# pengpeng-yu/FastPCC

Hardware: AMD Instinct MI355X
Metric: encode+decode Mpoints/sec, lossy_coord_v2 baseline_r1 (stream of 16-frame batches, 2 in flight; one frame at a time = value_one_frame) (higher is better)
Workload: dtype f32; 1 GPU; lossy_coord_v2/baseline_r1 inference, 997645-voxel 1024^3 body-surface frames (cfg#2), seeded random-init weights; one step = a batch of 16 such frames per GPU (15966320 voxels) through compress_many + decompress_many = ONE network traversal over the batch, 16 independent streams; 2 batch(es) in flight per GPU; parallelism=single GPU, 2 batches in flight per GPU on one stream (fastpcc_amd/serving.py), batch_clouds=16, frames_in_flight=2, named_stages=False, bytes=143901, coder_handover_retries=0

## Files before the change

fastpcc_amd/csrc/hip/conv.hip:

```cpp
#include "conv_common.h"
#include <atomic>
#include <cstdlib>

namespace fpcc {
namespace {

template <int NBT, int CH, int WM, int WN>
struct MfmaCfg {
    static constexpr int C_OUT = 32 * NBT;
    static constexpr int TM = 32 * WM;
    static constexpr int NBW = NBT / WN;
    static constexpr int THREADS = 64 * WM * WN;
    static constexpr int G8 = CH / 8;
    static constexpr int W_TOTAL = CH * C_OUT / 4;
    static constexpr int W_PIECES = (W_TOTAL + THREADS - 1) / THREADS;
    static_assert(NBT % WN == 0, "column blocks must divide over the waves");
};

template <typename C, int CH>
__device__ __forceinline__ void fetch_a(const ConvArgs &a, const int32_t *nbr_rows, int cc, int li, int lh,
                                        f32x4 (&ra)[C::G8]) {
    const bool in_x1 = cc * CH < a.c1;
    const float *xb = in_x1 ? a.x1 + cc * CH : a.x2 + (cc * CH - a.c1);
    const int64_t ld = in_x1 ? a.ld1 : a.ld2;
// ... 610 lines not shown
            for (int r = 0; r < 16; ++r) acc[rb][nb][r] = 0.0f;

    const int n_stages = __popc(wmask) * n_chunks;
    if (n_stages > 0) {
        const int64_t chunk_floats = (int64_t)G8 * nbt * 256;
        const float *wp_g = wp + (int64_t)g * a.n_off * n_chunks * chunk_floats + ((int64_t)cg * 2) * 256 + lane * 4;
        const float *const zero = (const float *)g_zero_row + 4 * lh;
        const float *const x1b = a.x1 + 4 * lh, *const x2b = a.x2 ? a.x2 + 4 * lh : zero;
        const int64_t ld1 = a.ld1, ld2 = a.ld2;
        const int n1 = a.c1 / CH;
        const float *a1[2], *a2[2], *bpk;
        int step[2];
        auto set_offset = [&](int k) {
#pragma unroll
            for (int rb = 0; rb < 2; ++rb) {
                const int32_t idx = s_nbr[k * 64 + 32 * rb + li];
                const int32_t neg = idx >> 31;
                const uint64_t m = (uint64_t)(int64_t)neg, z = reinterpret_cast<uint64_t>(zero) & m;
                const int64_t row = idx & ~neg;
                a1[rb] = reinterpret_cast<const float *>((reinterpret_cast<uint64_t>(x1b + row * ld1) & ~m) | z);
                a2[rb] = reinterpret_cast<const float *>((reinterpret_cast<uint64_t>(x2b + row * ld2) & ~m) | z);
                step[rb] = CH & ~neg;
            }
            bpk = wp_g + (int64_t)k * n_chunks * chunk_floats;
        };
        unsigned rest = wmask;
        int cc_f = 0;
        set_offset(__ffs(rest) - 1);
        const float *ap[2], *bp;
        auto next_stage = [&]() {
            const bool in1 = cc_f < n1;
            const int c = in1 ? cc_f : cc_f - n1;
            ap[0] = (in1 ? a1[0] : a2[0]) + c * step[0];
            ap[1] = (in1 ? a1[1] : a2[1]) + c * step[1];
            bp = bpk + cc_f * chunk_floats;
            if (cc_f + 1 < n_chunks) {
                ++cc_f;
            } else {
                const unsigned r2 = rest & (rest - 1);
                if (r2) { rest = r2; cc_f = 0; set_offset(__ffs(r2) - 1); }
            }
        };
        f32x4 ra[2][G8], rbv[G8][2];
        next_stage();
#pragma unroll
        for (int g8 = 0; g8 < G8; ++g8) {
            __builtin_amdgcn_sched_barrier(0);
            ra[0][g8] = *reinterpret_cast<const f32x4 *>(ap[0] + 8 * g8);
            __builtin_amdgcn_sched_barrier(0);
            ra[1][g8] = *reinterpret_cast<const f32x4 *>(ap[1] + 8 * g8);
#pragma unroll
            for (int nb = 0; nb < 2; ++nb) {
                __builtin_amdgcn_sched_barrier(0);
                rbv[g8][nb] = *reinterpret_cast<const f32x4 *>(bp + ((int64_t)g8 * nbt + nb) * 256);
            }
        }
        __builtin_amdgcn_sched_barrier(0);
        for (int s = 0; s < n_stages; ++s) {
            next_stage();
            __builtin_amdgcn_sched_barrier(SB);
#pragma unroll
            for (int g8 = 0; g8 < G8; ++g8) {
                const f32x4 av0 = ra[0][g8], av1 = ra[1][g8];
                const f32x4 b0 = rbv[g8][0], b1 = rbv[g8][1];
#define FPCC_STEP(c)                                                                                     \
                acc[0][0] = __builtin_amdgcn_mfma_f32_32x32x2f32(av0.c, b0.c, acc[0][0], 0, 0, 0);       \
                acc[0][1] = __builtin_amdgcn_mfma_f32_32x32x2f32(av0.c, b1.c, acc[0][1], 0, 0, 0);       \
                acc[1][0] = __builtin_amdgcn_mfma_f32_32x32x2f32(av1.c, b0.c, acc[1][0], 0, 0, 0);       \
                acc[1][1] = __builtin_amdgcn_mfma_f32_32x32x2f32(av1.c, b1.c, acc[1][1], 0, 0, 0);
                FPCC_STEP(x) FPCC_STEP(y) FPCC_STEP(z) FPCC_STEP(w)
#undef FPCC_STEP
                __builtin_amdgcn_sched_barrier(SB);
                ra[0][g8] = *reinterpret_cast<const f32x4 *>(ap[0] + 8 * g8);
                __builtin_amdgcn_sched_barrier(SB);
                ra[1][g8] = *reinterpret_cast<const f32x4 *>(ap[1] + 8 * g8);
#pragma unroll
                for (int nb = 0; nb < 2; ++nb) {
                    __builtin_amdgcn_sched_barrier(SB);
                    rbv[g8][nb] = *reinterpret_cast<const f32x4 *>(bp + ((int64_t)g8 * nbt + nb) * 256);
                }
                __builtin_amdgcn_sched_barrier(SB);
            }
        }
    }

    const float slope = (a.act == FPCC_ACT_PRELU && a.slope) ? a.slope[0] : 0.0f;
    float bias2[2];
#pragma unroll
    for (int nb = 0; nb < 2; ++nb) bias2[nb] = a.bias ? a.bias[32 * ((int)cg * 2 + nb) + li] : 0.0f;
#pragma unroll
    for (int rb = 0; rb < 2; ++rb) {
        int64_t dsts[16];
#pragma unroll
        for (int reg = 0; reg < 16; ++reg) {
            const int64_t o = __shfl(my_row, 32 * rb + (reg & 3) + 8 * (reg >> 2) + 4 * lh);
            dsts[reg] = o < 0 ? -1 : a.out_map ? (int64_t)a.out_map[o * a.om_os + g * a.om_gs] : o * a.groups + g;
        }
#pragma unroll
        for (int reg = 0; reg < 16; ++reg) {
            const int64_t dst = dsts[reg];
            if (dst < 0) continue;
#pragma unroll
            for (int nb = 0; nb < 2; ++nb)
                a.out[dst * a.ldo + 32 * ((int)cg * 2 + nb) + li] = finish(acc[rb][nb][reg], bias2[nb], a.act, slope, a.clip);
        }
    }
}

__global__ __launch_bounds__(256) void k_pack_weights(const float *__restrict__ w, int64_t n_mats, int c_in, int c_out,
                                                      float *__restrict__ wp) {
    const int64_t e = (int64_t)blockIdx.x * 256 + threadIdx.x;
    const int64_t per_mat = (int64_t)c_in * c_out;
    if (e >= n_mats * per_mat) return;
    const int nbt = c_out / 32;
    const int64_t m = e / per_mat;
    int64_t r = e - m * per_mat;
    const int j = (int)(r & 3); r >>= 2;
    const int i = (int)(r & 31); r >>= 5;
    const int h = (int)(r & 1); r >>= 1;
    const int nb = (int)(r % nbt); r /= nbt;
    const int g8 = (int)(r & 3); r >>= 2;
    const int cc = (int)r;
    wp[e] = w[m * per_mat + (int64_t)(32 * cc + 8 * g8 + 4 * h + j) * c_out + 32 * nb + i];
}

inline bool aligned16(const void *p) { return (reinterpret_cast<uintptr_t>(p) & 15) == 0; }

int mfma_chunk(int c1, int c2, int c_out) {
    if (c_out != 32 && c_out != 64 && c_out != 128) return 0;
    const int c_in = c1 + c2;
    if (c_in % 32 == 0 && c1 % 32 == 0) return 32;
    if (c_in % 16 == 0 && c1 % 16 == 0) return 16;
    return 0;
}

int knob(int k);

template <int NBT, int CH, int WM, int WN>
int launch_mfma_cfg(ConvArgs a, hipStream_t s) {
    constexpr int TM = 32 * WM;
    const unsigned tiles = (unsigned)((a.n_out + TM - 1) / TM);
    const dim3 grid(tiles, a.groups), block(64 * WM * WN);
    const int dbg = (NBT == 4 && CH == 32) ? knob(3) : 0;
    if (dbg == 1) hipLaunchKernelGGL((k_conv_mfma<NBT, CH, WM, WN, 1>), grid, block, 0, s, a);
    else if (dbg == 2) hipLaunchKernelGGL((k_conv_mfma<NBT, CH, WM, WN, 2>), grid, block, 0, s, a);
    else if (dbg == 3) hipLaunchKernelGGL((k_conv_mfma<NBT, CH, WM, WN, 3>), grid, block, 0, s, a);
    else if (dbg == 4) hipLaunchKernelGGL((k_conv_mfma<NBT, CH, WM, WN, 4>), grid, block, 0, s, a);
    else if (dbg == 7) hipLaunchKernelGGL((k_conv_mfma<NBT, CH, WM, WN, 7>), grid, block, 0, s, a);
    else hipLaunchKernelGGL((k_conv_mfma<NBT, CH, WM, WN>), grid, block, 0, s, a);
    return check_hip(hipGetLastError(), "k_conv_mfma");
}

enum { kKnobWaveOn = 0, kKnobWaveNbw = 1, kKnobWaveSb = 2, kKnobWaveDbg = 3, kKnobGroupedFoldRows = 4, kKnobMfmaCfg = 5, kKnobPointwiseRows = 6,
       kKnobGroupedOff = 7, kKnobGroupedNbw = 8, kKnobWave22Rows = 9, kKnobLdsRows = 10, kKnobLdsRowBlocks = 11, kKnobPersist = 12, kKnobCount = 13 };
int g_knob[kKnobCount] = {-1, -1, -1, -1, -1, -1, -1, -1, -1, -1, -1, -1, -1};
int knob(int k) {
    if (g_knob[k] < 0) {
        static const char *names[kKnobCount] = {"FPCC_CONV_WAVE", "FPCC_WAVE_NBW", "FPCC_WAVE_SB", "FPCC_WAVE_DBG", "FPCC_GROUPED_FOLD_ROWS",
                                                "FPCC_MFMA_TILE", "FPCC_POINTWISE_MIN_ROWS", "", "FPCC_GROUPED_NBW",
                                                "FPCC_WAVE22_MIN_ROWS", "FPCC_LDS_MIN_ROWS", "FPCC_LDS_ROW_BLOCKS",
                                                "FPCC_CONV_PERSIST"};
        static const int defaults[kKnobCount] = {1, 0, 1, 0, 100 * 1024, 0, 32 * 1024, 0, 0, 0, 0, 2, 0};
        const char *e = k == kKnobGroupedOff ? nullptr : getenv(names[k]);
        g_knob[k] = e ? atoi(e) : defaults[k];
    }
    return g_knob[k];
}

template <int NBT, int CH>
int launch_mfma(const ConvArgs &a, hipStream_t s) {
    const int forced = knob(kKnobMfmaCfg) - 1;
    const int64_t work = a.n_out * a.groups;
    constexpr int WNS = NBT >= 2 ? 2 : 1;
    const int cfg = forced >= 0 ? forced : (NBT <= 2 && work >= 128 * 1024) ? 0 : work >= 32 * 1024 ? 1 : 2;
    if (cfg == 0) return launch_mfma_cfg<NBT, CH, 4, 1>(a, s);
    if (cfg == 1) return launch_mfma_cfg<NBT, CH, 2, WNS>(a, s);
    return launch_mfma_cfg<NBT, CH, 1, NBT>(a, s);
}

__global__ __launch_bounds__(256) void k_conv_c1_pointwise(ConvArgs a) {
    const int64_t e = (int64_t)blockIdx.x * 256 + threadIdx.x;
    if (e >= a.n_out * a.c_out) return;
    const int64_t o = e / a.c_out;
    const int j = (int)(e - o * a.c_out);
    const float slope = (a.act == FPCC_ACT_PRELU && a.slope) ? a.slope[0] : 0.0f;
    a.out[o * a.ldo + j] = finish(fmaf(a.x1[o * a.ld1], a.w[j], 0.0f), a.bias ? a.bias[j] : 0.0f, a.act, slope, a.clip);
}

template <int NBW>
int launch_wave_cfg(const ConvArgs &a, const float *wp, int nbt, hipStream_t s) {
    const int64_t row_blocks = (a.n_out + 31) / 32;
    const int64_t units = row_blocks * (nbt / NBW);
    if (units > 0x7fffffffll) return fail_arg("conv_f32: too many work units");
    const dim3 grid((unsigned)((units + 3) / 4), a.groups);
    const int dbg = knob(kKnobWaveDbg);
    if (dbg == 1) hipLaunchKernelGGL((k_conv_wave<NBW, 32, 0x6, 1>), grid, dim3(256), 0, s, a, wp, nbt, (unsigned)units);
    else if (dbg == 2) hipLaunchKernelGGL((k_conv_wave<NBW, 32, 0x6, 2>), grid, dim3(256), 0, s, a, wp, nbt, (unsigned)units);
    else if (dbg == 3) hipLaunchKernelGGL((k_conv_wave<NBW, 32, 0x6, 3>), grid, dim3(256), 0, s, a, wp, nbt, (unsigned)units);
    else if (knob(kKnobWaveSb)) hipLaunchKernelGGL((k_conv_wave<NBW, 32, 0x6>), grid, dim3(256), 0, s, a, wp, nbt, (unsigned)units);
    else hipLaunchKernelGGL((k_conv_wave<NBW, 32, 0>), grid, dim3(256), 0, s, a, wp, nbt, (unsigned)units);
    return check_hip(hipGetLastError(), "k_conv_wave");
}

constexpr int kMaxDevices = 16;
inline int current_device() {
    int dev = 0;
    return (hipGetDevice(&dev) == hipSuccess && dev >= 0 && dev < kMaxDevices) ? dev : -1;
}
int cu_count() {
    static std::atomic<int> cached[kMaxDevices];
    const int dev = current_device();
    if (dev < 0) return 256;
    int n = cached[dev].load(std::memory_order_relaxed);
    if (n == 0) {
        hipDeviceProp_t prop;
        n = (hipGetDeviceProperties(&prop, dev) == hipSuccess && prop.multiProcessorCount > 0) ? prop.multiProcessorCount : 256;
        cached[dev].store(n, std::memory_order_relaxed);
    }
    return n;
}

constexpr int kUnitCounters = 256;
__device__ unsigned g_unit_counters[kUnitCounters];
unsigned *next_unit_counter(unsigned start, hipStream_t s, int *rc) {
    static std::atomic<unsigned> seq{0};
    static std::atomic<unsigned *> bases[kMaxDevices];
    const int dev = current_device();
    if (dev < 0) {
        *rc = fail_arg("unit counters: no current device");
        return nullptr;
    }
    unsigned *base = bases[dev].load(std::memory_order_acquire);
    if (!base) {
        if (hipGetSymbolAddress(reinterpret_cast<void **>(&base), HIP_SYMBOL(g_unit_counters)) != hipSuccess) {
            *rc = check_hip(hipGetLastError(), "unit counters");
            return nullptr;
        }
        bases[dev].store(base, std::memory_order_release);
    }
    unsigned *c = base + (seq++ % kUnitCounters);
    *rc = check_hip(hipMemsetD32Async(reinterpret_cast<hipDeviceptr_t>(c), (int)start, 1, s), "unit counter fill");
    return c;
}

inline int64_t persist_slots() {
    const int v = knob(kKnobPersist);
    return v > 16 ? v : (int64_t)v * cu_count();
}
inline bool persist_ok(const ConvArgs &a) {
    return knob(kKnobPersist) > 0 && a.nbr && a.nbr_ks == 1 && (a.nbr_os & 3) == 0 && a.nbr_os >= ((a.n_off + 3) & ~3) &&
           (reinterpret_cast<uintptr_t>(a.nbr) & 15) == 0 && a.groups == 1;
}

template <int NBW>
int launch_grouped_cfg(const ConvArgs &a, const float *wp, int nbt, hipStream_t s) {
    const int64_t row_blocks = (a.n_out + 31) / 32;
    const int64_t units = row_blocks * (nbt / NBW);
    if (units > 0x7fffffffll) return fail_arg("conv_f32: too many work units");
    const int dbg = knob(kKnobWaveDbg);
    const int64_t slots = persist_slots();
    if (dbg == 0 && persist_ok(a) && units > slots) {
        int rc = FPCC_OK;
        unsigned *counter = next_unit_counter((unsigned)slots, s, &rc);
        if (rc != FPCC_OK) return rc;
        hipLaunchKernelGGL((k_conv_wave<NBW, 32, 0x6, 0, 4, false, false, true>), dim3((unsigned)slots, 1), dim3(256), 0, s, a, wp, nbt, (unsigned)units,
                           counter);
        return check_hip(hipGetLastError(), "k_conv_wave(grouped, persistent)");
    }
    if (dbg == 16)
        hipLaunchKernelGGL((k_conv_wave<NBW, 32, 0x6, 16, 4>), dim3((unsigned)units, a.groups), dim3(256), 0, s, a, wp, nbt, (unsigned)units);
    else if (NBW == 1 && dbg == 17)
        hipLaunchKernelGGL((k_conv_wave<1, 32, 0x6, 17, 4>), dim3((unsigned)units, a.groups), dim3(256), 0, s, a, wp, nbt, (unsigned)units);
    else if (NBW == 1 && dbg == 18)
        hipLaunchKernelGGL((k_conv_wave<1, 32, 0x6, 18, 4>), dim3((unsigned)units, a.groups), dim3(256), 0, s, a, wp, nbt, (unsigned)units);
    else if (NBW == 1 && dbg == 19)
        hipLaunchKernelGGL((k_conv_wave<1, 32, 0x6, 19, 4>), dim3((unsigned)units, a.groups), dim3(256), 0, s, a, wp, nbt, (unsigned)units);
    else
        hipLaunchKernelGGL((k_conv_wave<NBW, 32, 0x6, 0, 4>), dim3((unsigned)units, a.groups), dim3(256), 0, s, a, wp, nbt, (unsigned)units);
    return check_hip(hipGetLastError(), "k_conv_wave(grouped)");
}

template <int NBW>
int launch_folded_cfg(const ConvArgs &a, const float *wp, int nbt, hipStream_t s) {
    const int64_t units = ((a.n_out + 31) / 32) * (nbt / NBW);
    if (units > 0x7fffffffll) return fail_arg("conv_f32: too many work units");
    const int64_t slots = persist_slots();
    if (knob(kKnobWaveDbg) == 0 && persist_ok(a) && (units + 3) / 4 > slots) {
        int rc = FPCC_OK;
        unsigned *counter = next_unit_counter((unsigned)(4 * slots), s, &rc);
        if (rc != FPCC_OK) return rc;
        hipLaunchKernelGGL((k_conv_wave<NBW, 32, 0x6, 0, 1, true, false, true>), dim3((unsigned)slots, 1), dim3(256), 0, s, a, wp, nbt, (unsigned)units,
                           counter);
        return check_hip(hipGetLastError(), "k_conv_wave(folded, persistent)");
    }
    if (knob(kKnobWaveDbg) == 64) {
        hipLaunchKernelGGL((k_conv_wave<NBW, 32, 0x6, 0, 1, true, false, false, 1>), dim3((unsigned)units, a.groups), dim3(64), 0, s, a, wp, nbt,
                           (unsigned)units);
        return check_hip(hipGetLastError(), "k_conv_wave(folded, one wave per workgroup)");
    }
    if (NBW == 2 && knob(kKnobWaveDbg) == 32)
        hipLaunchKernelGGL((k_conv_wave<2, 32, 0x6, 0, 1, true, true>), dim3((unsigned)((units + 3) / 4), a.groups), dim3(256), 0, s, a, wp, nbt,
                           (unsigned)units);
    else
        hipLaunchKernelGGL((k_conv_wave<NBW, 32, 0x6, 0, 1, true>), dim3((unsigned)((units + 3) / 4), a.groups), dim3(256), 0, s, a, wp, nbt,
                           (unsigned)units);
    return check_hip(hipGetLastError(), "k_conv_wave(folded)");
}

int launch_grouped(const ConvArgs &a, const float *wp, hipStream_t s) {
    const int nbt = a.c_out / 32;
    const int64_t lds_rows = knob(kKnobLdsRows);
    if (lds_rows > 0 && a.n_out >= lds_rows) {
        const int rc = launch_conv_lds(a, wp, knob(kKnobLdsRowBlocks), knob(kKnobWaveDbg) & 63, s);
        if (rc != -1) return rc;
    }
    const int64_t fold_rows = knob(kKnobGroupedFoldRows);
    if (fold_rows > 0 && a.n_out >= fold_rows && knob(kKnobGroupedNbw) <= 0)
        return nbt % 2 == 0 ? launch_folded_cfg<2>(a, wp, nbt, s) : launch_folded_cfg<1>(a, wp, nbt, s);
    int nbw = knob(kKnobGroupedNbw);
    if (nbw <= 0) nbw = a.n_out >= 40 * 1024 ? 2 : 1;
    while (nbw > nbt || nbt % nbw) nbw >>= 1;
    return nbw == 2 ? launch_grouped_cfg<2>(a, wp, nbt, s) : launch_grouped_cfg<1>(a, wp, nbt, s);
}

int launch_wave22(const ConvArgs &a, const float *wp, int nbt, hipStream_t s) {
    const int64_t units = ((a.n_out + 63) / 64) * (nbt / 2);
    if (units > 0x7fffffffll) return fail_arg("conv_f32: too many work units");
    const dim3 grid((unsigned)((units + 3) / 4), a.groups);
    if (knob(kKnobWaveSb)) hipLaunchKernelGGL((k_conv_wave22<0x6>), grid, dim3(256), 0, s, a, wp, nbt, (unsigned)units);
    else hipLaunchKernelGGL((k_conv_wave22<0>), grid, dim3(256), 0, s, a, wp, nbt, (unsigned)units);
    return check_hip(hipGetLastError(), "k_conv_wave22");
}

int launch_wave(const ConvArgs &a, const float *wp, hipStream_t s) {
    const int nbt = a.c_out / 32;
    const int64_t work = a.n_out * a.groups;
    const int64_t rows22 = knob(kKnobWave22Rows);
    if (rows22 > 0 && a.n_off > 1 && nbt % 2 == 0 && work >= rows22 && knob(kKnobWaveNbw) <= 0) return launch_wave22(a, wp, nbt, s);
    int nbw = knob(kKnobWaveNbw);
    if (nbw <= 0) nbw = work >= 32 * 1024 ? 2 : 1;
    while (nbw > nbt || nbt % nbw) nbw >>= 1;
    if (nbw >= 4) return launch_wave_cfg<4>(a, wp, nbt, s);
    if (nbw == 2) return launch_wave_cfg<2>(a, wp, nbt, s);
    return launch_wave_cfg<1>(a, wp, nbt, s);
}


template <int NBW, int NCH, int DBG = 0>
__global__ __launch_bounds__(256, 2) void k_pointwise_wave(ConvArgs a, const float *__restrict__ wp, int nbt, unsigned n_row_blocks,
                                                           unsigned waves_per_cg) {
    constexpr int AC = NCH < 4 ? NCH : 4;
    constexpr int TW = 32 * NBW + 4;
    __shared__ float s_tile[4][32 * TW];
    const int lane = threadIdx.x & 63, wv = threadIdx.x >> 6;
    const int li = lane & 31, lh = lane >> 5;
    const unsigned n_cg = (unsigned)(nbt / NBW);
    const unsigned w = blockIdx.x * 4u + (unsigned)wv;
    const unsigned cg = w % n_cg, slot = w / n_cg;
    if (slot >= waves_per_cg) return;

    f32x4 rb[NCH][4][NBW];
    {
        const float *wpl = wp + ((int64_t)cg * NBW) * 256 + lane * 4;
#pragma unroll
        for (int cc = 0; cc < NCH; ++cc)
#pragma unroll
            for (int g8 = 0; g8 < 4; ++g8)
#pragma unroll
                for (int nb = 0; nb < NBW; ++nb)
                    rb[cc][g8][nb] = *reinterpret_cast<const f32x4 *>(wpl + (((int64_t)cc * 4 + g8) * nbt + nb) * 256);
    }
    const int n1 = a.c1 / 32;
    const float slope = (a.act == FPCC_ACT_PRELU && a.slope) ? a.slope[0] : 0.0f;
    float bias[NBW];
#pragma unroll
    for (int nb = 0; nb < NBW; ++nb) bias[nb] = a.bias ? a.bias[32 * ((int)cg * NBW + nb) + li] : 0.0f;

    auto row_ptrs = [&](unsigned rbk, const float *&q1, const float *&q2) {
        int64_t row = (int64_t)rbk * 32 + li;
        if (row >= a.n_out) row = a.n_out - 1;
        if (DBG & 1) row = lane & 1;
        q1 = a.x1 + row * a.ld1 + 4 * lh;
        q2 = a.x2 ? a.x2 + row * a.ld2 + 4 * lh : q1;
    };
    auto fetch = [&](const float *q1, const float *q2, int cc, int g8) -> f32x4 {
        if (DBG & 8) { const float v = (float)(lane + g8 + cc); return f32x4{v, v + 1.0f, v + 2.0f, v + 3.0f}; }
        const float *src = cc < n1 ? q1 + 32 * cc : q2 + 32 * (cc - n1);
        return *reinterpret_cast<const f32x4 *>(src + 8 * g8);
    };
    const float *c1p, *c2p, *n1p, *n2p;
    row_ptrs(slot, c1p, c2p);
    f32x4 ra[AC][4];
#pragma unroll
    for (int c = 0; c < AC; ++c)
#pragma unroll
        for (int g8 = 0; g8 < 4; ++g8) {
            __builtin_amdgcn_sched_barrier(0);
            ra[c][g8] = fetch(c1p, c2p, c, g8);
        }
    __builtin_amdgcn_sched_barrier(0);
    for (unsigned rbk = slot; rbk < n_row_blocks; rbk += waves_per_cg) {
        const int64_t row0 = (int64_t)rbk * 32;
        row_ptrs(rbk + waves_per_cg, n1p, n2p);
        f32x16 acc[NBW];
#pragma unroll
        for (int nb = 0; nb < NBW; ++nb)
#pragma unroll
            for (int r = 0; r < 16; ++r) acc[nb][r] = 0.0f;
#pragma unroll
        for (int cc = 0; cc < NCH; ++cc) {
            constexpr int kNone = 0;
            (void)kNone;
            const int sl = cc % AC;
            const bool wraps = cc + AC >= NCH;
            const int cn = (cc + AC) % NCH;
#pragma unroll
            for (int g8 = 0; g8 < 4; ++g8) {
                const f32x4 av = ra[sl][g8];
#pragma unroll
                for (int nb = 0; nb < NBW; ++nb) acc[nb] = __builtin_amdgcn_mfma_f32_32x32x2f32(av.x, rb[cc][g8][nb].x, acc[nb], 0, 0, 0);
#pragma unroll
                for (int nb = 0; nb < NBW; ++nb) acc[nb] = __builtin_amdgcn_mfma_f32_32x32x2f32(av.y, rb[cc][g8][nb].y, acc[nb], 0, 0, 0);
#pragma unroll
                for (int nb = 0; nb < NBW; ++nb) acc[nb] = __builtin_amdgcn_mfma_f32_32x32x2f32(av.z, rb[cc][g8][nb].z, acc[nb], 0, 0, 0);
#pragma unroll
                for (int nb = 0; nb < NBW; ++nb) acc[nb] = __builtin_amdgcn_mfma_f32_32x32x2f32(av.w, rb[cc][g8][nb].w, acc[nb], 0, 0, 0);
                __builtin_amdgcn_sched_barrier(0x6);
                ra[sl][g8] = wraps ? fetch(n1p, n2p, cn, g8) : fetch(c1p, c2p, cn, g8);
                __builtin_amdgcn_sched_barrier(0x6);
            }
        }
        c1p = n1p;
        c2p = n2p;
        float *tile = s_tile[wv];
#pragma unroll
        for (int reg = 0; reg < 16; ++reg) {
            const int r = (reg & 3) + 8 * (reg >> 2) + 4 * lh;
#pragma unroll
            for (int nb = 0; nb < NBW; ++nb) tile[r * TW + 32 * nb + li] = finish(acc[nb][reg], bias[nb], a.act, slope, a.clip);
        }
        __builtin_amdgcn_wave_barrier();
        constexpr int LPR = 8 * NBW;
        constexpr int RPI = 64 / LPR;
        const int qr = lane / LPR, qc = lane % LPR;
#pragma unroll
        for (int r0 = 0; r0 < 32; r0 += RPI) {
            const int r = r0 + qr;
            const f32x4 v = *reinterpret_cast<const f32x4 *>(tile + r * TW + 4 * qc);
            const int64_t o = row0 + r;
            if (o < a.n_out && !((DBG & 4) && v.x != 12345.678f))
                *reinterpret_cast<f32x4 *>(a.out + o * a.ldo + 32 * (int)cg * NBW + 4 * qc) = v;
        }
        __builtin_amdgcn_wave_barrier();
    }
}


template <int NBW, int NCH>
int launch_pointwise_cfg(const ConvArgs &a, const float *wp, int nbt, hipStream_t s) {
    const unsigned row_blocks = (unsigned)((a.n_out + 31) / 32);
    const unsigned n_cg = (unsigned)(nbt / NBW);
    unsigned waves_per_cg = (256u * 4u * 2u) / n_cg;
    if (waves_per_cg > row_blocks) waves_per_cg = row_blocks;
    const unsigned waves = waves_per_cg * n_cg;
    const int dbg = (NBW == 2 && NCH == 4) ? knob(kKnobWaveDbg) : 0;
    if (dbg == 1) hipLaunchKernelGGL((k_pointwise_wave<NBW, NCH, 1>), dim3((waves + 3) / 4), dim3(256), 0, s, a, wp, nbt, row_blocks, waves_per_cg);
// ... 582 lines not shown
```

fastpcc_amd/csrc/hip/conv_common.h:

```cpp
#pragma once
#include "common.h"

namespace fpcc {

typedef float f32x16 __attribute__((ext_vector_type(16)));
typedef float f32x4 __attribute__((ext_vector_type(4)));

struct ConvArgs {
    const float *x1; int c1; int ld1;
    const float *x2; int c2; int ld2;
    const int32_t *nbr; int n_off; int64_t nbr_ks; int64_t nbr_os;
    const float *w; const float *bias; int c_out; int groups;
    const int32_t *out_map; int64_t om_os; int64_t om_gs; float *out; int ldo; int64_t n_out;
    int act; const float *slope; float clip;
    const int32_t *row_order;
};

static __device__ float g_zero_row[64];

__device__ __forceinline__ float finish(float v, float b, int act, float slope, float clip) {
    v = v + b;
    if (act == FPCC_ACT_PRELU) v = v < 0.0f ? v * slope : v;
    else if (act == FPCC_ACT_RELU) v = v < 0.0f ? 0.0f : v;
    if (clip > 0.0f) v = fminf(fmaxf(v, -clip), clip);
    return v;
}

__device__ __forceinline__ unsigned xcd_remap(unsigned bid, unsigned n) {
    const unsigned q = n / 8, r = n % 8, x = bid % 8;
    return (x < r ? x * (q + 1) : r * (q + 1) + (x - r) * q) + bid / 8;
}

constexpr int kMaxOffsets = 27;

typedef int i32x4 __attribute__((ext_vector_type(4)));

__device__ __forceinline__ bool table_is_row_major(const ConvArgs &a) {
    return a.nbr && a.nbr_ks == 1 && (a.nbr_os & 3) == 0 && a.nbr_os >= ((a.n_off + 3) & ~3) && (reinterpret_cast<uintptr_t>(a.nbr) & 15) == 0;
}

__host__ __device__ __forceinline__ int offset_group_begin(int g, int n_off) { return (g * n_off + 3) / 4; }
__host__ __device__ __forceinline__ int offset_group_of(int k, int n_off) {
    return (k >= offset_group_begin(1, n_off)) + (k >= offset_group_begin(2, n_off)) + (k >= offset_group_begin(3, n_off));
}

constexpr int kStampSlots = 48;
static __device__ unsigned long long *g_stamp_buf = nullptr;
static __device__ long long g_stamp_cap = 0;
__device__ __forceinline__ void stamp_lds(unsigned long long *slot) {
    const unsigned long long t = __builtin_amdgcn_s_memtime();
    const unsigned addr = (unsigned)(uintptr_t)slot;
    asm volatile("s_mov_b64 exec, 1\n\tds_write_b64 %0, %1\n\ts_mov_b64 exec, -1" ::"v"(addr), "v"(t) : "memory");
}
__device__ __forceinline__ void stamp_lds_realtime(unsigned long long *slot) {
    const unsigned long long t = __builtin_amdgcn_s_memrealtime();
    const unsigned addr = (unsigned)(uintptr_t)slot;
    asm volatile("s_mov_b64 exec, 1\n\tds_write_b64 %0, %1\n\ts_mov_b64 exec, -1" ::"v"(addr), "v"(t) : "memory");
}
int set_lds_stamp_buffer(unsigned long long *buf, long long cap);

int launch_conv_lds(const ConvArgs &a, const float *wp, int row_blocks, int dbg, hipStream_t s);

}
```

fastpcc_amd/hipops.py:

```python
import collections
import ctypes as C
import functools
from typing import List, Optional, Tuple

import torch

from . import _native

_vp, _i64, _i32, _f32 = C.c_void_p, C.c_int64, C.c_int, C.c_float

ACT_NONE, ACT_PRELU, ACT_RELU = 0, 1, 2

_SIGS = {
    'fpcc_morton3d_encode': (_i32, [_vp, _i64, _i64, _i32, _i32, _i32, _vp, _vp]),
    'fpcc_hilbert3d_encode': (_i32, [_vp, _i64, _i64, _i32, _i32, _i32, _i32, _vp, _vp]),
    'fpcc_keys_from_coords': (_i32, [_vp, _i64, _i32, _i32, _vp, _vp]),
    'fpcc_coords_from_keys': (_i32, [_vp, _i64, _i32, _i32, _vp, _vp, _vp]),
    'fpcc_sort_keys': (_i64, [_vp, _i64, _i32, _vp, _vp, _vp, _i64, _vp]),
    'fpcc_unique_keys': (_i64, [_vp, _i64, _vp, _vp, _vp, _vp, _i64, _vp]),
    'fpcc_coarsen': (_i64, [_vp, _i64, _vp, _vp, _vp, _vp, _vp, _i64, _vp]),
    'fpcc_octree_level': (_i64, [_vp, _i64, _i64, _i32, _vp, _vp, _vp, _vp, _i64, _vp, _vp, _i64, _vp]),
    'fpcc_level_histogram': (_i64, [_vp, _i64, _i32, _vp, _vp]),
    'fpcc_level_histogram_clouds': (_i64, [_vp, _i64, _i32, _i32, _i32, _vp, _vp]),
    'fpcc_refine': (_i64, [_vp, _i64, _vp, _vp, _vp, _vp, _vp, _vp, _i64, _vp]),
# ... 279 lines not shown
    if n == 0:
        return [0] * levels
    hist = torch.empty(levels + 1, dtype=torch.int32, device=keys.device)
    _ok(lib().fpcc_level_histogram(_dev(keys, torch.int64, 'keys'), n, levels, hist.data_ptr(), _stream()))
    h = hist.tolist()
    out, acc = [], 0
    for t in range(levels, 0, -1):
        acc += h[t]
        out.append(1 + acc)
    return out[::-1]


def level_counts_clouds(keys: torch.Tensor, levels: int, cloud_shift: int, n_clouds: int) -> List[List[int]]:
    n = keys.shape[0]
    hist = torch.empty((n_clouds, levels + 2), dtype=torch.int32, device=keys.device)
    _ok(lib().fpcc_level_histogram_clouds(_dev(keys, torch.int64, 'keys'), n, levels, int(cloud_shift), int(n_clouds),
                                          hist.data_ptr(), _stream()))
    h = hist.tolist()
    if sum(row[levels + 1] for row in h) != n:
        raise ValueError(f'a key carries a cloud index outside the batch of {n_clouds}: either the batch column is wrong or a coordinate '
                         f'(after subtracting its cloud\'s minimum) needs more than {cloud_shift // 3} bits per axis -- the Morton code of a '
                         f'cloud is {cloud_shift} bits wide (resolutions up to {1 << (cloud_shift // 3)})')
    out = [[0] * n_clouds for _ in range(levels + 1)]
    for c, row in enumerate(h):
        if row[levels + 1] and row[levels + 1] != 1 + sum(row[:levels + 1]):
            raise ValueError(f'cloud {c}: the keys are not unique ({row[levels + 1]} keys, {1 + sum(row[:levels + 1])} distinct)')
        out[0][c] = row[levels + 1]
        acc = 0
        for t in range(levels, 0, -1):
            acc += row[t]
            out[t][c] = acc + (1 if row[levels + 1] else 0)
    return out


def refine(pkeys: torch.Tensor, mask: torch.Tensor):
    m = pkeys.shape[0]
    dev = pkeys.device
    if mask.dtype == torch.bool:
        mask = mask.view(torch.uint8)
    if mask.numel() != 8 * m:
        raise ValueError('mask must have 8 entries per parent')
    keys = torch.empty(8 * m, dtype=torch.int64, device=dev)
    parent_of = torch.empty(8 * m, dtype=torch.int32, device=dev)
    child_row = torch.empty((m, 8), dtype=torch.int32, device=dev)
    count = torch.empty(1, dtype=torch.int32, device=dev)
    L = lib()
    ws, need = _ws(lambda: L.fpcc_refine(None, m, None, None, None, None, None, None, 0, None), dev)
    _ok(L.fpcc_refine(_dev(pkeys, torch.int64, 'pkeys'), m, _dev(mask, torch.uint8, 'mask'), keys.data_ptr(),
                      parent_of.data_ptr(), child_row.data_ptr(), count.data_ptr(), ws.data_ptr(), need, _stream()))
    return keys, parent_of, child_row, count


def nbr27_search(keys: torch.Tensor, bits: int) -> torch.Tensor:
    n = keys.shape[0]
    nbr = torch.empty((27, n), dtype=torch.int32, device=keys.device)
    _ok(lib().fpcc_nbr27_search(_dev(keys, torch.int64, 'keys'), n, bits, nbr.data_ptr(), _stream()))
    return nbr


def nbr27_from_parent(keys: Optional[torch.Tensor], parent_of: Optional[torch.Tensor], parent_nbr: torch.Tensor,
                      child_row: Optional[torch.Tensor], n: Optional[int] = None) -> torch.Tensor:
    m = parent_nbr.shape[1]
    if keys is None:
        n = 8 * m if n is None else n
    else:
        n = keys.shape[0]
    nbr = torch.empty((27, n), dtype=torch.int32, device=parent_nbr.device)
    _ok(lib().fpcc_nbr27_from_parent(_dev(keys, torch.int64, 'keys', True), _dev(parent_of, torch.int32, 'parent_of', True),
                                     n, _dev(parent_nbr, torch.int32, 'parent_nbr'), m,
                                     _dev(child_row, torch.int32, 'child_row', True), nbr.data_ptr(), _stream()))
    return nbr


def nbr27_from_parent_ex(keys: Optional[torch.Tensor], parent_of: Optional[torch.Tensor], parent_nbr: torch.Tensor,
                         child_row: Optional[torch.Tensor], n: Optional[int] = None):
    m = parent_nbr.shape[1]
    n = (8 * m if n is None else n) if keys is None else keys.shape[0]
    dev = parent_nbr.device
    nbr = torch.empty((27, n), dtype=torch.int32, device=dev)
    rows = torch.empty((n, 32), dtype=torch.int32, device=dev)
    masks = torch.empty(n, dtype=torch.int32, device=dev)
    _ok(lib().fpcc_nbr27_from_parent_ex(_dev(keys, torch.int64, 'keys', True), _dev(parent_of, torch.int32, 'parent_of', True),
                                        n, _dev(parent_nbr, torch.int32, 'parent_nbr'), m,
                                        _dev(child_row, torch.int32, 'child_row', True), nbr.data_ptr(), rows.data_ptr(),
                                        masks.data_ptr(), _stream()))
    return nbr, rows, masks


def gather_table_rows(rows: torch.Tensor, order: torch.Tensor) -> torch.Tensor:
    n, ld = rows.shape
    out = torch.empty_like(rows)
    _ok(lib().fpcc_gather_table_rows_i32(_dev(rows, torch.int32, 'rows'), ld, _dev(order, torch.int32, 'order'), n, out.data_ptr(), _stream()))
    return out


def mask27_from_parent(keys: Optional[torch.Tensor], parent_of: Optional[torch.Tensor], parent_nbr: torch.Tensor,
                       child_row: Optional[torch.Tensor], n: Optional[int] = None) -> torch.Tensor:
    m = parent_nbr.shape[1]
    n = (8 * m if n is None else n) if keys is None else keys.shape[0]
    masks = torch.empty(n, dtype=torch.int32, device=parent_nbr.device)
    _ok(lib().fpcc_mask27_from_parent(_dev(keys, torch.int64, 'keys', True), _dev(parent_of, torch.int32, 'parent_of', True),
                                      n, _dev(parent_nbr, torch.int32, 'parent_nbr'), m,
                                      _dev(child_row, torch.int32, 'child_row', True), masks.data_ptr(), _stream()))
    return masks


def conv_ones_k3(masks: torch.Tensor, w: torch.Tensor, c_out: int, *, bias: Optional[torch.Tensor] = None, act: int = 0,
                 slope: Optional[torch.Tensor] = None, clip: float = 0.0) -> torch.Tensor:
    n = masks.shape[0]
    if w.numel() != 27 * c_out or not w.is_contiguous():
        raise ValueError('weights must be contiguous [27, 1, c_out]')
    out = torch.empty((n, c_out), dtype=torch.float32, device=masks.device)
    _ok(lib().fpcc_conv_ones_k3_f32(_dev(masks, torch.int32, 'masks'), n, _dev(w, torch.float32, 'w'),
                                    _dev(bias, torch.float32, 'bias', True), c_out, act, _dev(slope, torch.float32, 'slope', True),
                                    float(clip), out.data_ptr(), c_out, _stream()))
    return out



def _rows2d(t: torch.Tensor, name: str):
    if t.dim() != 2 or t.dtype != torch.float32 or not t.is_cuda or t.stride(1) != 1:
        raise TypeError(f'{name} must be a 2-D float32 GPU tensor with unit column stride')
    return t.data_ptr(), t.shape[1], (t.stride(0) if t.shape[0] > 1 else max(t.shape[1], t.stride(0)))


_PACKED: 'collections.OrderedDict' = collections.OrderedDict()
_PACKED_MAX = 1024


def packed_weights(w: torch.Tensor, c1: int, c2: int, c_out: int, n_offsets: int, groups: int, fresh: bool = False) -> Optional[torch.Tensor]:
    if not lib().fpcc_conv_packed_floats(c1, c2, c_out, n_offsets, groups):
        return None
    if fresh:
        out = torch.empty(w.numel(), dtype=torch.float32, device=w.device)
        _ok(lib().fpcc_conv_pack_weights_f32(w.data_ptr(), groups * n_offsets, c1 + c2, c_out, out.data_ptr(), _stream()))
        return out
    key = (w.data_ptr(), w.numel(), c1 + c2, c_out)
    ent = _PACKED.get(key)
    if ent is not None and ent[1] == w._version:
        _PACKED.move_to_end(key)
        return ent[2]
    out = torch.empty(w.numel(), dtype=torch.float32, device=w.device)
    _ok(lib().fpcc_conv_pack_weights_f32(w.data_ptr(), groups * n_offsets, c1 + c2, c_out, out.data_ptr(), _stream()))
    _PACKED[key] = (w, w._version, out)
    while len(_PACKED) > _PACKED_MAX:
        _PACKED.popitem(last=False)
    return out


KNOB_WAVE_ON, KNOB_WAVE_NBW, KNOB_WAVE_SB, KNOB_WAVE_DBG, KNOB_MFMA_TILE, KNOB_POINTWISE_ROWS = 0, 1, 2, 3, 5, 6
KNOB_GROUPED_FOLD_ROWS = 4
KNOB_GROUPED_OFF, KNOB_GROUPED_NBW, KNOB_WAVE22_ROWS = 7, 8, 9
KNOB_PERSIST = 12
KNOB_LDS_ROWS, KNOB_LDS_ROW_BLOCKS = 10, 11


def numerics_version() -> int:
    return lib().fpcc_numerics_version()


def clock_probe(out2: torch.Tensor, spin_us: int = 20) -> None:
    _ok(lib().fpcc_clock_probe(_dev(out2, torch.int64, 'out2'), int(spin_us), _stream()))


def transpose_table(table: torch.Tensor, ld: int = 32) -> torch.Tensor:
    k, n = table.shape
    out = torch.empty((n, ld), dtype=torch.int32, device=table.device)
    _ok(lib().fpcc_transpose_table_i32(_dev(table, torch.int32, 'table', n == 0), k, n, out.data_ptr(), ld, _stream()))
    return out


def conv_debug_stamps(buf: Optional[torch.Tensor]) -> None:
    if buf is None:
        _ok(lib().fpcc_conv_debug_stamps(None, 0))
    else:
        _ok(lib().fpcc_conv_debug_stamps(_dev(buf, torch.int64, 'buf'), buf.numel()))


def conv_i8_debug_stamps(buf: Optional[torch.Tensor]) -> None:
    if buf is None:
        _ok(lib().fpcc_conv_i8_debug_stamps(None, 0))
    else:
        _ok(lib().fpcc_conv_i8_debug_stamps(_dev(buf, torch.int64, 'buf'), buf.numel()))


def conv_set_tuning(which: int, value: int) -> int:
    before = _ok(lib().fpcc_conv_set_tuning(int(which), int(value)))
    conv_order.cache_clear()
    return before


CONV_TRACE = None
TRACE_LOCK = __import__('threading').RLock()
CLOCK_HOOK = None
_EVENT_POOL: list = []
_trace_tls = __import__('threading').local()


def set_thread_trace(trace) -> None:
    global _n_thread_traces
    had = getattr(_trace_tls, 'trace', None) is not None
    _trace_tls.trace = trace
    with TRACE_LOCK:
        _n_thread_traces += (trace is not None) - had


_n_thread_traces = 0


def _untraced_launch(fn, call) -> None:
    if _n_thread_traces:
        with TRACE_LOCK:
            _ok(fn(*call))
    else:
        _ok(fn(*call))


def _current_trace():
    t = getattr(_trace_tls, 'trace', None)
    return t if t is not None else CONV_TRACE


def reserve_trace_events(n: int) -> None:
    while len(_EVENT_POOL) < n:
        ev = torch.cuda.Event(enable_timing=True)
        ev.record()
        _EVENT_POOL.append(ev)


def _trace_event():
    if _EVENT_POOL:
        return _EVENT_POOL.pop()
    ev = torch.cuda.Event(enable_timing=True)
    ev.record()
    return ev


def _traced_launch(trace: list, fn, call, info) -> None:
    with TRACE_LOCK:
        ev0, ev1 = _trace_event(), _trace_event()
        if CLOCK_HOOK is not None:
            ev0.record()
            CLOCK_HOOK(ev0, info.get('n_out', 0), info.get('n_offsets', 1))
            _ok(fn(*call))
            ev1.record()
        else:
            _ok(lib().fpcc_time_next_launch(ev0.cuda_event, ev1.cuda_event))
            try:
                _ok(fn(*call))
            except BaseException:
                lib().fpcc_time_next_launch(None, None)
                raise
        trace.append((ev0, ev1, info))


def conv_f32(x1: torch.Tensor, w: torch.Tensor, c_out: int, n_out: int, *, x2: Optional[torch.Tensor] = None,
             nbr: Optional[torch.Tensor] = None, n_offsets: int = 1, nbr_ks: int = 0, nbr_os: int = 1,
             bias: Optional[torch.Tensor] = None, groups: int = 1, out_map: Optional[torch.Tensor] = None,
             om_os: int = 0, om_gs: int = 1, out: Optional[torch.Tensor] = None, out_rows: Optional[int] = None,
             act: int = ACT_NONE, slope: Optional[torch.Tensor] = None, clip: float = 0.0,
             row_order: Optional[torch.Tensor] = None, pack: bool = False) -> torch.Tensor:
    p1, c1, ld1 = _rows2d(x1, 'x1')
    if x2 is not None:
        p2, c2, ld2 = _rows2d(x2, 'x2')
    else:
        p2, c2, ld2 = None, 0, 0
    if w.dtype != torch.float32 or not w.is_cuda or not w.is_contiguous() or \
            w.numel() != groups * n_offsets * (c1 + c2) * c_out:
        raise ValueError(f'weights must be contiguous fp32 [{groups},{n_offsets},{c1 + c2},{c_out}], got {tuple(w.shape)}')
    if out is None:
        rows = out_rows if out_rows is not None else n_out * groups
        out = torch.empty((rows, c_out), dtype=torch.float32, device=x1.device)
    po, co, ldo = _rows2d(out, 'out')
    if co != c_out:
        raise ValueError('output width mismatch')
    if om_os == 0:
        om_os = groups
    ws, ws_bytes = None, 0
    wp = packed_weights(w, c1, c2, c_out, n_offsets, groups, fresh=(pack == 'fresh')) if pack else None
    if wp is None and nbr is not None and n_offsets >= 8:
        ws_bytes = lib().fpcc_conv_f32_ws_bytes(c1, c2, c_out, n_offsets, groups, n_out)
        if ws_bytes:
            ws = torch.empty(ws_bytes // 4, dtype=torch.float32, device=x1.device)
    fn = lib().fpcc_conv_f32_pk
    call = (p1, c1, ld1, p2, c2, ld2, _dev(nbr, torch.int32, 'nbr', True), n_offsets, nbr_ks, nbr_os,
            w.data_ptr(), None if wp is None else wp.data_ptr(),
            _dev(bias, torch.float32, 'bias', True), c_out, groups,
            _dev(out_map, torch.int32, 'out_map', True), om_os, om_gs, po, ldo, n_out, act,
            _dev(slope, torch.float32, 'slope', True), float(clip),
            _dev(row_order, torch.int32, 'row_order', True),
            None if ws is None else ws.data_ptr(), ws_bytes, _stream())
    trace = _current_trace()
    if trace is None:
        _untraced_launch(fn, call)
        return out
    _traced_launch(trace, fn, call, {'mfma': bool(conv_order(c1, c2, c_out, n_offsets, groups, n_out)), 'c_in': c1 + c2, 'c_out': c_out,
                                     'n_out': n_out, 'groups': groups, 'n_offsets': n_offsets, 'nbr': nbr,
                                     'nbr_ks': nbr_ks, 'nbr_os': nbr_os})
    return out


class _MlpLayer(C.Structure):
    _fields_ = [('w', _vp), ('w_packed', _vp), ('bias', _vp), ('slope', _vp), ('c_out', _i32), ('act', _i32), ('clip', _f32)]


class _MlpChain(C.Structure):
# ... 733 lines not shown
```

Before: 89.19 Mpoints/s.

## Add paired-row-block grouped conv kernel for large 27-offset layers

Adds a new grouped sparse-conv kernel where each wave computes two 32-row blocks against two 32-column output blocks. A-fragments are reused across both column blocks and B-fragments across both row blocks, and the next stage's operands are software-pipelined. It is used by default for layers with at least 200K output rows, 27 offsets and an even column-block count. It takes over from the folded path there. The cost is higher register pressure (4 accumulators plus fold sums) and possible lower occupancy.

```diff
diff --git a/fastpcc_amd/csrc/hip/conv.hip b/fastpcc_amd/csrc/hip/conv.hip
--- a/fastpcc_amd/csrc/hip/conv.hip
+++ b/fastpcc_amd/csrc/hip/conv.hip
@@ -786,15 +786,16 @@
 }
 
 enum { kKnobWaveOn = 0, kKnobWaveNbw = 1, kKnobWaveSb = 2, kKnobWaveDbg = 3, kKnobGroupedFoldRows = 4, kKnobMfmaCfg = 5, kKnobPointwiseRows = 6,
-       kKnobGroupedOff = 7, kKnobGroupedNbw = 8, kKnobWave22Rows = 9, kKnobLdsRows = 10, kKnobLdsRowBlocks = 11, kKnobPersist = 12, kKnobCount = 13 };
-int g_knob[kKnobCount] = {-1, -1, -1, -1, -1, -1, -1, -1, -1, -1, -1, -1, -1};
+       kKnobGroupedOff = 7, kKnobGroupedNbw = 8, kKnobWave22Rows = 9, kKnobLdsRows = 10, kKnobLdsRowBlocks = 11, kKnobPersist = 12,
+       kKnobPairRows = 13, kKnobPairSkip = 14, kKnobCount = 15 };
+int g_knob[kKnobCount] = {-1, -1, -1, -1, -1, -1, -1, -1, -1, -1, -1, -1, -1, -1, -1};
 int knob(int k) {
     if (g_knob[k] < 0) {
         static const char *names[kKnobCount] = {"FPCC_CONV_WAVE", "FPCC_WAVE_NBW", "FPCC_WAVE_SB", "FPCC_WAVE_DBG", "FPCC_GROUPED_FOLD_ROWS",
                                                 "FPCC_MFMA_TILE", "FPCC_POINTWISE_MIN_ROWS", "", "FPCC_GROUPED_NBW",
                                                 "FPCC_WAVE22_MIN_ROWS", "FPCC_LDS_MIN_ROWS", "FPCC_LDS_ROW_BLOCKS",
-                                                "FPCC_CONV_PERSIST"};
-        static const int defaults[kKnobCount] = {1, 0, 1, 0, 100 * 1024, 0, 32 * 1024, 0, 0, 0, 0, 2, 0};
+                                                "FPCC_CONV_PERSIST", "FPCC_PAIR_FOLD_ROWS", "FPCC_PAIR_SKIP"};
+        static const int defaults[kKnobCount] = {1, 0, 1, 0, 100 * 1024, 0, 32 * 1024, 0, 0, 0, 0, 2, 0, 200 * 1024, 0};
         const char *e = k == kKnobGroupedOff ? nullptr : getenv(names[k]);
         g_knob[k] = e ? atoi(e) : defaults[k];
     }
@@ -946,6 +947,11 @@
     const int64_t lds_rows = knob(kKnobLdsRows);
     if (lds_rows > 0 && a.n_out >= lds_rows) {
         const int rc = launch_conv_lds(a, wp, knob(kKnobLdsRowBlocks), knob(kKnobWaveDbg) & 63, s);
+        if (rc != -1) return rc;
+    }
+    const int64_t pair_rows = knob(kKnobPairRows);
+    if (pair_rows > 0 && a.n_out >= pair_rows && a.n_off == 27 && nbt % 2 == 0 && knob(kKnobGroupedNbw) <= 0 && knob(kKnobWaveDbg) == 0) {
+        const int rc = launch_conv_pair(a, wp, knob(kKnobPairSkip), s);
         if (rc != -1) return rc;
     }
     const int64_t fold_rows = knob(kKnobGroupedFoldRows);
diff --git a/fastpcc_amd/csrc/hip/conv_common.h b/fastpcc_amd/csrc/hip/conv_common.h
--- a/fastpcc_amd/csrc/hip/conv_common.h
+++ b/fastpcc_amd/csrc/hip/conv_common.h
@@ -61,4 +61,6 @@
 
 int launch_conv_lds(const ConvArgs &a, const float *wp, int row_blocks, int dbg, hipStream_t s);
 
+int launch_conv_pair(const ConvArgs &a, const float *wp, int skip, hipStream_t s);
+
 }
diff --git a/fastpcc_amd/csrc/hip/conv_pair.hip b/fastpcc_amd/csrc/hip/conv_pair.hip
--- /dev/null
+++ b/fastpcc_amd/csrc/hip/conv_pair.hip
@@ -0,0 +1,254 @@
+#include "conv_common.h"
+
+namespace fpcc {
+namespace {
+
+template <int SB, bool SKIP>
+__global__ __launch_bounds__(256, 2) void k_conv_pair(ConvArgs a, const float *__restrict__ wp, int nbt, unsigned n_units) {
+    constexpr int CH = 32, G8 = 4;
+    __shared__ int32_t s_nbr_all[4][32 * 64];
+
+    const int lane = threadIdx.x & 63, wv = __builtin_amdgcn_readfirstlane(threadIdx.x >> 6);
+    const int li = lane & 31, lh = lane >> 5;
+    const unsigned n_cg = (unsigned)(nbt / 2);
+    const unsigned blk = a.row_order ? blockIdx.x : xcd_remap(blockIdx.x, gridDim.x);
+    const unsigned unit = blk * 4u + (unsigned)wv;
+    if (unit >= n_units) return;
+    const unsigned pr = unit / n_cg, cg = unit - pr * n_cg;
+    const int64_t row0 = (int64_t)pr * 64;
+    const int g = blockIdx.y;
+    const int c_in = a.c1 + a.c2;
+    const int n_chunks = c_in / CH;
+    int32_t *s_nbr = s_nbr_all[wv];
+
+    int32_t my_row[2] = {-1, -1};
+    unsigned bmask[2] = {0u, 0u};
+    if (table_is_row_major(a)) {
+        i32x4 q[2][4];
+        const int last_piece = (a.n_off - 1) >> 2;
+#pragma unroll
+        for (int rb = 0; rb < 2; ++rb) {
+            const int64_t p = row0 + 32 * rb + li;
+            const int64_t pc = p < a.n_out ? p : a.n_out - 1;
+            const int32_t o = a.row_order ? a.row_order[pc] : (int32_t)pc;
+            my_row[rb] = p < a.n_out ? o : -1;
+            const i32x4 *rowp = reinterpret_cast<const i32x4 *>(a.nbr + (a.row_order ? pc : (int64_t)o) * a.nbr_os);
+#pragma unroll
+            for (int j = 0; j < 4; ++j) q[rb][j] = rowp[min(4 * lh + j, last_piece)];
+        }
+#pragma unroll
+        for (int rb = 0; rb < 2; ++rb)
+#pragma unroll
+            for (int j = 0; j < 4; ++j)
+#pragma unroll
+                for (int e = 0; e < 4; ++e) {
+                    const int k = 16 * lh + 4 * j + e;
+                    const int k0 = 4 * j + e;
+                    const int32_t v = (k < a.n_off && my_row[rb] >= 0) ? q[rb][j][e] : -1;
+                    s_nbr[k * 64 + 32 * rb + li] = v;
+                    const unsigned long long b = __ballot(v >= 0);
+                    if (b & 0xffffffffull) bmask[rb] |= 1u << k0;
+                    if (b >> 32) bmask[rb] |= 1u << (k0 + 16);
+                }
+    } else {
+#pragma unroll
+        for (int rb = 0; rb < 2; ++rb) {
+            const int64_t p = row0 + 32 * rb + li;
+            if (p < a.n_out) my_row[rb] = a.row_order ? a.row_order[p] : (int32_t)p;
+            for (int k0 = 0; k0 < a.n_off; k0 += 2) {
+                const int k = k0 + lh;
+                int32_t v = -1;
+                if (k < a.n_off && my_row[rb] >= 0) v = a.nbr ? a.nbr[(int64_t)k * a.nbr_ks + (int64_t)my_row[rb] * a.nbr_os] : my_row[rb];
+                if (k < a.n_off) s_nbr[k * 64 + 32 * rb + li] = v;
+                const unsigned long long b = __ballot(v >= 0);
+                if (b & 0xffffffffull) bmask[rb] |= 1u << k0;
+                if (b >> 32) bmask[rb] |= 1u << (k0 + 1);
+            }
+        }
+    }
+    __builtin_amdgcn_wave_barrier();
+    const unsigned m0 = __builtin_amdgcn_readfirstlane(bmask[0]), m1 = __builtin_amdgcn_readfirstlane(bmask[1]);
+    const unsigned wmask = m0 | m1;
+
+    f32x16 acc[2][2];
+#pragma unroll
+    for (int rb = 0; rb < 2; ++rb)
+#pragma unroll
+        for (int nb = 0; nb < 2; ++nb)
+#pragma unroll
+            for (int r = 0; r < 16; ++r) acc[rb][nb][r] = 0.0f;
+
+    f32x16 tsum[2][2];
+    int n_folded = 0, cur_g = 0;
+    auto fold_acc = [&]() {
+#pragma unroll
+        for (int rb = 0; rb < 2; ++rb)
+#pragma unroll
+            for (int nb = 0; nb < 2; ++nb)
+#pragma unroll
+                for (int r = 0; r < 16; ++r) {
+                    tsum[rb][nb][r] = n_folded ? tsum[rb][nb][r] + acc[rb][nb][r] : acc[rb][nb][r];
+                    acc[rb][nb][r] = 0.0f;
+                }
+        ++n_folded;
+    };
+    auto fold_zero = [&]() {
+#pragma unroll
+        for (int rb = 0; rb < 2; ++rb)
+#pragma unroll
+            for (int nb = 0; nb < 2; ++nb)
+#pragma unroll
+                for (int r = 0; r < 16; ++r) tsum[rb][nb][r] = n_folded ? tsum[rb][nb][r] + 0.0f : 0.0f;
+        ++n_folded;
+    };
+    unsigned rest_c = wmask;
+    int cc_c = 0;
+    unsigned which = 3;
+    if (wmask) {
+        cur_g = offset_group_of(__ffs(wmask) - 1, a.n_off);
+        for (int gz = 0; gz < cur_g; ++gz) fold_zero();
+    }
+
+    const int n_stages = __popc(wmask) * n_chunks;
+    if (n_stages > 0) {
+        const int64_t chunk_floats = (int64_t)G8 * nbt * 256;
+        const float *wp_g = wp + (int64_t)g * a.n_off * n_chunks * chunk_floats + ((int64_t)cg * 2) * 256 + lane * 4;
+        const float *const zero = (const float *)g_zero_row + 4 * lh;
+        const float *const x1b = a.x1 + 4 * lh, *const x2b = a.x2 ? a.x2 + 4 * lh : zero;
+        const int64_t ld1 = a.ld1, ld2 = a.ld2;
+        const int n1 = a.c1 / CH;
+        const float *a1[2], *a2[2], *bpk;
+        int step[2];
+        auto set_offset = [&](int k) {
+#pragma unroll
+            for (int rb = 0; rb < 2; ++rb) {
+                const int32_t idx = s_nbr[k * 64 + 32 * rb + li];
+                const int32_t neg = idx >> 31;
+                const uint64_t m = (uint64_t)(int64_t)neg, z = reinterpret_cast<uint64_t>(zero) & m;
+                const int64_t row = idx & ~neg;
+                a1[rb] = reinterpret_cast<const float *>((reinterpret_cast<uint64_t>(x1b + row * ld1) & ~m) | z);
+                a2[rb] = reinterpret_cast<const float *>((reinterpret_cast<uint64_t>(x2b + row * ld2) & ~m) | z);
+                step[rb] = CH & ~neg;
+            }
+            bpk = wp_g + (int64_t)k * n_chunks * chunk_floats;
+        };
+        unsigned rest = wmask;
+        int cc_f = 0;
+        set_offset(__ffs(rest) - 1);
+        const float *ap[2], *bp;
+        auto next_stage = [&]() {
+            const bool in1 = cc_f < n1;
+            const int c = in1 ? cc_f : cc_f - n1;
+            ap[0] = (in1 ? a1[0] : a2[0]) + c * step[0];
+            ap[1] = (in1 ? a1[1] : a2[1]) + c * step[1];
+            bp = bpk + cc_f * chunk_floats;
+            if (cc_f + 1 < n_chunks) {
+                ++cc_f;
+            } else {
+                const unsigned r2 = rest & (rest - 1);
+                if (r2) { rest = r2; cc_f = 0; set_offset(__ffs(r2) - 1); }
+            }
+        };
+        f32x4 ra[2][G8], rbv[G8][2];
+        next_stage();
+#pragma unroll
+        for (int g8 = 0; g8 < G8; ++g8) {
+#pragma unroll
+            for (int rb = 0; rb < 2; ++rb) {
+                __builtin_amdgcn_sched_barrier(0);
+                ra[rb][g8] = *reinterpret_cast<const f32x4 *>(ap[rb] + 8 * g8);
+            }
+#pragma unroll
+            for (int nb = 0; nb < 2; ++nb) {
+                __builtin_amdgcn_sched_barrier(0);
+                rbv[g8][nb] = *reinterpret_cast<const f32x4 *>(bp + ((int64_t)g8 * nbt + nb) * 256);
+            }
+        }
+        __builtin_amdgcn_sched_barrier(0);
+        for (int s = 0; s < n_stages; ++s) {
+            if (cc_c == 0) {
+                const int kc = __ffs(rest_c) - 1;
+                const int gk = offset_group_of(kc, a.n_off);
+                if (gk != cur_g) {
+                    fold_acc();
+                    for (int gz = cur_g + 1; gz < gk; ++gz) fold_zero();
+                    cur_g = gk;
+                }
+                if (SKIP) which = ((m0 >> kc) & 1u) | (((m1 >> kc) & 1u) << 1);
+            }
+            if (++cc_c == n_chunks) { cc_c = 0; rest_c &= rest_c - 1; }
+            next_stage();
+            __builtin_amdgcn_sched_barrier(SB);
+#pragma unroll
+            for (int g8 = 0; g8 < G8; ++g8) {
+                const f32x4 av0 = ra[0][g8], av1 = ra[1][g8];
+                const f32x4 b0 = rbv[g8][0], b1 = rbv[g8][1];
+#define FPCC_ROW(r, av, c)                                                                                   \
+                acc[r][0] = __builtin_amdgcn_mfma_f32_32x32x2f32(av.c, b0.c, acc[r][0], 0, 0, 0);            \
+                acc[r][1] = __builtin_amdgcn_mfma_f32_32x32x2f32(av.c, b1.c, acc[r][1], 0, 0, 0);
+                if (!SKIP) {
+                    FPCC_ROW(0, av0, x) FPCC_ROW(1, av1, x)
+                    FPCC_ROW(0, av0, y) FPCC_ROW(1, av1, y)
+                    FPCC_ROW(0, av0, z) FPCC_ROW(1, av1, z)
+                    FPCC_ROW(0, av0, w) FPCC_ROW(1, av1, w)
+                } else {
+                    if (which & 1u) { FPCC_ROW(0, av0, x) FPCC_ROW(0, av0, y) FPCC_ROW(0, av0, z) FPCC_ROW(0, av0, w) }
+                    if (which & 2u) { FPCC_ROW(1, av1, x) FPCC_ROW(1, av1, y) FPCC_ROW(1, av1, z) FPCC_ROW(1, av1, w) }
+                }
+#undef FPCC_ROW
+                __builtin_amdgcn_sched_barrier(SB);
+#pragma unroll
+                for (int rb = 0; rb < 2; ++rb) {
+                    ra[rb][g8] = *reinterpret_cast<const f32x4 *>(ap[rb] + 8 * g8);
+                    __builtin_amdgcn_sched_barrier(SB);
+                }
+#pragma unroll
+                for (int nb = 0; nb < 2; ++nb) {
+                    rbv[g8][nb] = *reinterpret_cast<const f32x4 *>(bp + ((int64_t)g8 * nbt + nb) * 256);
+                    __builtin_amdgcn_sched_barrier(SB);
+                }
+            }
+        }
+    }
+
+    if (wmask) { fold_acc(); ++cur_g; }
+    for (int gz = cur_g; gz < 4; ++gz) fold_zero();
+
+    const float slope = (a.act == FPCC_ACT_PRELU && a.slope) ? a.slope[0] : 0.0f;
+    float bias2[2];
+#pragma unroll
+    for (int nb = 0; nb < 2; ++nb) bias2[nb] = a.bias ? a.bias[32 * ((int)cg * 2 + nb) + li] : 0.0f;
+    int64_t dsts[2][16];
+#pragma unroll
+    for (int rb = 0; rb < 2; ++rb)
+#pragma unroll
+        for (int reg = 0; reg < 16; ++reg) {
+            const int64_t o = __shfl(my_row[rb], (reg & 3) + 8 * (reg >> 2) + 4 * lh);
+            dsts[rb][reg] = o < 0 ? -1 : a.out_map ? (int64_t)a.out_map[o * a.om_os + g * a.om_gs] : o * a.groups + g;
+        }
+#pragma unroll
+    for (int rb = 0; rb < 2; ++rb)
+#pragma unroll
+        for (int reg = 0; reg < 16; ++reg) {
+            const int64_t dst = dsts[rb][reg];
+            if (dst < 0) continue;
+#pragma unroll
+            for (int nb = 0; nb < 2; ++nb)
+                a.out[dst * a.ldo + 32 * ((int)cg * 2 + nb) + li] = finish(tsum[rb][nb][reg], bias2[nb], a.act, slope, a.clip);
+        }
+}
+
+}
+
+int launch_conv_pair(const ConvArgs &a, const float *wp, int skip, hipStream_t s) {
+    const int nbt = a.c_out / 32;
+    if (nbt % 2 || !a.nbr || a.n_off > kMaxOffsets || (a.c1 + a.c2) % 32 || a.c1 % 32) return -1;
+    const int64_t units = ((a.n_out + 63) / 64) * (nbt / 2);
+    if (units > 0x7fffffffll) return fail_arg("conv_f32: too many work units");
+    const dim3 grid((unsigned)((units + 3) / 4), a.groups);
+    if (skip) hipLaunchKernelGGL((k_conv_pair<0x6, true>), grid, dim3(256), 0, s, a, wp, nbt, (unsigned)units);
+    else hipLaunchKernelGGL((k_conv_pair<0x6, false>), grid, dim3(256), 0, s, a, wp, nbt, (unsigned)units);
+    return check_hip(hipGetLastError(), "k_conv_pair");
+}
+
+}
diff --git a/fastpcc_amd/hipops.py b/fastpcc_amd/hipops.py
--- a/fastpcc_amd/hipops.py
+++ b/fastpcc_amd/hipops.py
@@ -455,6 +455,7 @@
 KNOB_GROUPED_FOLD_ROWS = 4
 KNOB_GROUPED_OFF, KNOB_GROUPED_NBW, KNOB_WAVE22_ROWS = 7, 8, 9
 KNOB_PERSIST = 12
+KNOB_PAIR_ROWS, KNOB_PAIR_SKIP = 13, 14
 KNOB_LDS_ROWS, KNOB_LDS_ROW_BLOCKS = 10, 11
 
 
```

Result: faster. 90.98 Mpoints/s (median of 6 runs) (+2.0%).
